# maxspahn/robot_mpcs

Measured on AMD Instinct MI355X. Metric: MPC solves/sec (batched) at N=30, pointRobot & panda; 1/2/4/8 MI355X, higher is better.
Workload: dtype f64; 1 GPU; BASELINE configs[1]: pointRobot N=30, batch=4096 random start/goal + 3 static obstacles; batch_per_gpu=4096, horizon=30, nvar=9, npar=38, nh=15, warm_start=current_state (cold multipliers, every step solves from scratch), parallelism=1 x independent shards, no data-path collective, streams_per_gpu=4, input_sets=6

## Files before the change

robot_mpcs_amd/csrc/rmpc_fused.hpp:

```cpp

constexpr int kFusedStages = 32;

struct FusedWs {
  double *p;
  double *z[2], *t[2], *lam[2], *nu[2];
  double *dz, *nunew, *gfa;
  double *grow[2], *Jq[2];
  double *wlam, *wnu, *wmu;
  double *R;
  double *KP;
  int *passes;
  int *lastp;
  int *order;
  int *ckey;
  long long *stamps;
  int rs, kps, nv, m, nx, npar, nhs, njqs;
};

#define GSYNC()                                              \
  do {                                                       \
    __builtin_amdgcn_fence(__ATOMIC_RELEASE, "wavefront");   \
    __builtin_amdgcn_s_waitcnt(0);                           \
    __builtin_amdgcn_wave_barrier();                         \
    __builtin_amdgcn_fence(__ATOMIC_ACQUIRE, "wavefront");   \
  } while (0)

#define RMPC_ONE_WAVE
#define RMPC_PHASE __noinline__ RMPC_ONE_WAVE
template <class C>
__device__ RMPC_PHASE bool fused_recursion_lds(const int N, const double dt, const double mu, const double cw, const int lane,
                                               ldouble *const work, ldouble *const slots, const StepOut<ldouble> so) {
  return riccati_recursion<C, kFusedStages, true, ldouble>(N, dt, mu, cw, lane, work, slots, nullptr, 0, so, slots);
}
template <class C>
__device__ RMPC_PHASE bool fused_recursion_mem(const int N, const double dt, const double mu, const double cw, const int lane,
                                               ldouble *const work, const gdouble *const grec, gdouble *const kpb,
                                               const int kps, const StepOut<gdouble> so) {
  return riccati_recursion<C, kFusedStages, false, gdouble, true>(N, dt, mu, cw, lane, work, grec, kpb, kps, so);
}

struct FusedPtrs {
  gdouble *pz[2], *pt[2], *pl[2], *pn[2], *pg[2], *pj[2], *pp, *pdz, *pnn, *pgf, *pwl, *pwn;
};
__device__ __forceinline__ FusedPtrs fused_ptrs(const FusedWs &F, size_t b) {
  asm volatile("" : "+v"(b));
  const size_t S = kFusedStages;
  FusedPtrs P;
  P.pz[0] = (gdouble *)F.z[0] + b * F.nv * S; P.pz[1] = (gdouble *)F.z[1] + b * F.nv * S;
  P.pt[0] = (gdouble *)F.t[0] + b * F.m * S; P.pt[1] = (gdouble *)F.t[1] + b * F.m * S;
  P.pl[0] = (gdouble *)F.lam[0] + b * F.m * S; P.pl[1] = (gdouble *)F.lam[1] + b * F.m * S;
  P.pn[0] = (gdouble *)F.nu[0] + b * F.nx * S; P.pn[1] = (gdouble *)F.nu[1] + b * F.nx * S;
  P.pg[0] = (gdouble *)F.grow[0] + b * F.nhs * S; P.pg[1] = (gdouble *)F.grow[1] + b * F.nhs * S;
  P.pj[0] = (gdouble *)F.Jq[0] + b * F.njqs * S; P.pj[1] = (gdouble *)F.Jq[1] + b * F.njqs * S;
  P.pp = (gdouble *)F.p + b * F.npar * S;
  P.pdz = (gdouble *)F.dz + b * F.nv * S;
  P.pnn = (gdouble *)F.nunew + b * F.nx * S;
  P.pgf = (gdouble *)F.gfa + b * F.nv * S;
  P.pwl = (gdouble *)F.wlam + b * F.m * S;
  P.pwn = (gdouble *)F.wnu + b * F.nx * S;
  return P;
}

typedef const __attribute__((address_space(4))) FusedWs cFusedWs;
__device__ __forceinline__ cFusedWs *uniform_block(const FusedWs *p) {
  const unsigned long long a = (unsigned long long)p;
  const unsigned lo = __builtin_amdgcn_readfirstlane((unsigned)a), hi = __builtin_amdgcn_readfirstlane((unsigned)(a >> 32));
  return (cFusedWs *)(((unsigned long long)hi << 32) | lo);
}
__device__ __forceinline__ void load_block(FusedWs &F, const FusedWs *p) {
  static_assert(sizeof(FusedWs) % 8 == 0, "FusedWs is copied in 8-byte words");
  const __attribute__((address_space(4))) unsigned long long *src = (const __attribute__((address_space(4))) unsigned long long *)uniform_block(p);
  unsigned long long *dst = (unsigned long long *)&F;
#pragma unroll
  for (int i = 0; i < (int)(sizeof(FusedWs) / 8); i++) dst[i] = src[i];
}
struct FusedCur {
  gdouble *zc, *zn, *tc, *tn, *lc, *ln, *nc, *nn, *gc, *gn, *jc, *jn, *pp, *pdz, *pnn, *pgf, *pwl, *pwn;
};
__device__ __forceinline__ FusedCur fused_cur(const FusedWs &F, const size_t b, const int cur) {
  const FusedPtrs P = fused_ptrs(F, b);
  const bool c1 = cur != 0;
  FusedCur Q;
  Q.zc = c1 ? P.pz[1] : P.pz[0]; Q.zn = c1 ? P.pz[0] : P.pz[1];
  Q.tc = c1 ? P.pt[1] : P.pt[0]; Q.tn = c1 ? P.pt[0] : P.pt[1];
  Q.lc = c1 ? P.pl[1] : P.pl[0]; Q.ln = c1 ? P.pl[0] : P.pl[1];
  Q.nc = c1 ? P.pn[1] : P.pn[0]; Q.nn = c1 ? P.pn[0] : P.pn[1];
  Q.gc = c1 ? P.pg[1] : P.pg[0]; Q.gn = c1 ? P.pg[0] : P.pg[1];
  Q.jc = c1 ? P.pj[1] : P.pj[0]; Q.jn = c1 ? P.pj[0] : P.pj[1];
  Q.pp = P.pp; Q.pdz = P.pdz; Q.pnn = P.pnn; Q.pgf = P.pgf; Q.pwl = P.pwl; Q.pwn = P.pwn;
  return Q;
}

struct ArmBlock {
  FusedWs F;
  DevModel M;
};
typedef const __attribute__((address_space(4))) ArmBlock cArmBlock;
struct FusedHalf {
  double gphi_sum;
  int b, valid, retired, first, ipass, nextslot;
};
template <class V>
__device__ __forceinline__ V call_view(const FusedWs *Fp) {
  if constexpr (std::is_same<V, GView>::value) {
    const unsigned long long a = (unsigned long long)Fp;
    const unsigned lo = (unsigned)__builtin_amdgcn_readfirstlane((unsigned)a), hi = (unsigned)__builtin_amdgcn_readfirstlane((unsigned)(a >> 32));
    const unsigned long long u = ((unsigned long long)hi << 32) | lo;
    typedef const __attribute__((address_space(4))) ArmBlock cArmBlock;
    cArmBlock *const blk = (cArmBlock *)u;
    return GView(&blk->M, (GView::cTables *)(u - sizeof(DevTables)));
  } else {
    return V{};
  }
}
struct StepRes { double ap, ad, gp; };
template <class C, class V, int FIRSTC, bool REC_LDS>
__device__ __noinline__ RMPC_ONE_WAVE Partials fused_sweep_call(const FusedWs *Fp, const int N, const double dt, const int use_curv,
                                                  const size_t b, const int cur, const int k, ldouble *const slots,
                                                  const bool nostep, const double alpha, const double adual, const double mu,
                                                  const int warm) {
  using RP = typename std::conditional<REC_LDS, ldouble, gdouble>::type;
  constexpr int GS = FusedSlots<C>::GS, DZ_OFF = FusedSlots<C>::DZ_OFF, NV = C::NV;
  FusedWs F;
  load_block(F, Fp);
  const size_t S = kFusedStages;
  const FusedCur Pw = fused_cur(F, b, cur);
  SweepIO<RP> io;
  io.zc = Pw.zc; io.tc = Pw.tc; io.lc = Pw.lc; io.nc = Pw.nc;
  io.zn = Pw.zn; io.tn = Pw.tn; io.ln = Pw.ln; io.nn = Pw.nn;
  io.pp = Pw.pp; io.gro = Pw.gc; io.jqo = Pw.jc; io.grn = Pw.gn; io.jqn = Pw.jn;
  io.gfa = Pw.pgf;
  io.SS = S; io.loff = (unsigned)k; io.kstride = 1u;
  if constexpr (REC_LDS) {
    io.rec = slots + k * GS;
    io.dzp = slots + DZ_OFF; io.nup = slots + DZ_OFF + NV;
    io.SSd = 1; io.loffd = (unsigned)(k * GS); io.kstrided = (unsigned)GS;
  } else {
    io.rec = (gdouble *)F.R + (b * (size_t)N + k) * C::RS;
    io.dzp = Pw.pdz; io.nup = Pw.pnn;
    io.SSd = S; io.loffd = (unsigned)k; io.kstrided = 1u;
  }
  io.wl = Pw.pwl; io.wn = Pw.pwn; io.warm = warm;
  const SweepK sk = {N, dt, use_curv};
  const V v = call_view<V>(Fp);
  Partials q = {0, 0, 0, 0, 0, 0, 0, 0, 1e300, 0};
  sweep_body<C, -1, RP, V, FIRSTC>(sk, v, io, k, FIRSTC != 0, nostep, alpha, adual, mu, q);
  return q;
}
template <class C, class V, bool REC_LDS>
__device__ __noinline__ RMPC_ONE_WAVE StepRes fused_step_call(const FusedWs *Fp, const size_t b, const int cur, const int k,
                                                ldouble *const slots, const double mu) {
  using RP = typename std::conditional<REC_LDS, ldouble, gdouble>::type;
  constexpr int GS = FusedSlots<C>::GS, DZ_OFF = FusedSlots<C>::DZ_OFF;
  FusedWs F;
  load_block(F, Fp);
  const size_t S = kFusedStages;
  const FusedCur Ps = fused_cur(F, b, cur);
  StepIO<RP> io;
  io.zc = Ps.zc; io.tc = Ps.tc; io.lc = Ps.lc; io.grow = Ps.gc; io.Jq = Ps.jc;
  io.gfa = Ps.pgf;
  io.SS = S; io.loff = (unsigned)k;
  if constexpr (REC_LDS) { io.dz = slots + DZ_OFF; io.SSd = 1; io.loffd = (unsigned)(k * GS); }
  else { io.dz = Ps.pdz; io.SSd = S; io.loffd = (unsigned)k; }
  const V v = call_view<V>(Fp);
  StepRes r = {1.0, 1.0, 0.0};
  step_body<C, RP, V>(v, io, k, mu, r.ap, r.ad, r.gp);
  return r;
}

struct SweepStepOut { double f, th, lgs, sumc, badf, rstat, req, rineq, rcomp, minc, amin_p, amin_d, gphi;
#ifdef RMPC_STAMPS
  long long tk[6];
#endif
};
struct SweepStepRes { Partials q; double amin_p, amin_d, gphi; };
template <class C, class V, int FIRSTC>
__device__ __noinline__ RMPC_ONE_WAVE void fused_sweep_step_call(__attribute__((address_space(3))) SweepStepOut *const out,
                                                                 const FusedWs *Fp, const int N, const double dt, const int use_curv,
                                                           const size_t b, const int cur, const int k, ldouble *const slots,
                                                           const bool live, const bool nostep, const bool fresh, const int ls,
                                                           const double amin_p_in, const double amin_d_in, const double gphi_in,
                                                           const double mu, const int warm) {
  constexpr int GS = FusedSlots<C>::GS, DZ_OFF = FusedSlots<C>::DZ_OFF, NV = C::NV;
  FusedWs F;
  load_block(F, Fp);
  const size_t S = kFusedStages;
  const FusedCur Pw = fused_cur(F, b, cur);
  const V v{};
  SweepIO<ldouble> io;
  io.zc = Pw.zc; io.tc = Pw.tc; io.lc = Pw.lc; io.nc = Pw.nc;
  io.zn = Pw.zn; io.tn = Pw.tn; io.ln = Pw.ln; io.nn = Pw.nn;
  io.pp = Pw.pp; io.gro = Pw.gc; io.jqo = Pw.jc; io.grn = Pw.gn; io.jqn = Pw.jn;
  io.gfa = Pw.pgf;
  io.SS = S; io.loff = (unsigned)k; io.kstride = 1u;
  io.rec = slots + k * GS;
  io.dzp = slots + DZ_OFF; io.nup = slots + DZ_OFF + NV;
  io.SSd = 1; io.loffd = (unsigned)(k * GS); io.kstrided = (unsigned)GS;
  io.wl = Pw.pwl; io.wn = Pw.pwn; io.warm = warm;
  const SweepK sk = {N, dt, use_curv};
  SweepStepRes r;
  const Partials qn = {0, 0, 0, 0, 0, 0, 0, 0, 1e300, 0};
  r.q = qn;
  SecStamps st;
  st.start();
  if constexpr (FIRSTC != 0) {
    r.amin_p = amin_p_in; r.amin_d = amin_d_in; r.gphi = gphi_in;
    if (live) sweep_body<C, -1, ldouble, V, FIRSTC>(sk, v, io, k, true, nostep, 0.0, 0.0, mu, r.q);
  } else {
    SweepTop<C, V> top;
    StepRow<C> sl;
    if (live) sweep_body<C, -1, ldouble, V, 0, 1>(sk, v, io, k, false, nostep, 0.0, 0.0, mu, r.q, nullptr, &top, &sl);
    double ap = (fresh && live) ? sl.ap : 1.0, ad = (fresh && live) ? sl.ad : 1.0, gp = (fresh && live) ? sl.gphi : 0.0;
    st(4);
    {
      double rs1[1] = {gp}, rm0[1] = {0.0}, rn2[2] = {ap, ad};
      wave_reduce_many<kFusedStages>(rs1, rm0, rn2);
      gp = rs1[0]; ap = rn2[0]; ad = rn2[1];
    }
    st(5);
    r.amin_p = fresh ? fmin(amin_p_in, ap) : amin_p_in;
    r.amin_d = fresh ? fmin(amin_d_in, ad) : amin_d_in;
    r.gphi = fresh ? gp : gphi_in;
    const double alpha = nostep ? 0.0 : ldexp(r.amin_p, -ls), adual = nostep ? 0.0 : r.amin_d;
    if (live) sweep_body<C, -1, ldouble, V, 0, 2>(sk, v, io, k, false, nostep, alpha, adual, mu, r.q, nullptr, &top);
  }
  {
    const Partials &q = r.q;
    double rs5[5] = {q.f, q.th, q.logs, q.sumc, q.bad}, rm4[4] = {q.rstat, q.req, q.rineq, q.rcomp}, rn1[1] = {q.minc};
    wave_reduce_many<kFusedStages>(rs5, rm4, rn1);
    out->f = rs5[0]; out->th = rs5[1]; out->lgs = rs5[2]; out->sumc = rs5[3]; out->badf = rs5[4];
    out->rstat = rm4[0]; out->req = rm4[1]; out->rineq = rm4[2]; out->rcomp = rm4[3]; out->minc = rn1[0];
    out->amin_p = r.amin_p; out->amin_d = r.amin_d; out->gphi = r.gphi;
    st.get(q, 0, 4);
    if (k == 0) st.put(*out, 0, 6);
  }
}

template <class C, bool REC_LDS, class V>
__global__ __launch_bounds__(64, 1) __attribute__((amdgpu_waves_per_eu(1, 1), disable_tail_calls)) void k_fused(const DevModel M, const DevTables *__restrict__ Tp, const FusedWs F, const int B,
                                              const double *__restrict__ xinit, const double *__restrict__ x0,
                                              const double *__restrict__ params, double *__restrict__ zout,
                                              int *__restrict__ exitflag, int *__restrict__ iters_out,
                                              double *__restrict__ kkt, double *__restrict__ obj, const int max_passes,
                                              const int warm_mode, const int use_order, const int save_duals) {
  constexpr int LPI = kFusedStages;
  constexpr int IPW = 2;
  constexpr int NX = C::NX, NV = C::NV;
  using VC = typename std::conditional<V::SPEC, V, GView>::type;
  auto blk = [&]() __attribute__((always_inline)) -> cArmBlock * {
    unsigned long long a = (unsigned long long)(Tp + 1);
    asm volatile("" : "+s"(a));
    return (cArmBlock *)a;
  };
  const int half = threadIdx.x / LPI;
  const int k = threadIdx.x & (LPI - 1);
  const int N = blk()->M.N;
  const bool stage = k < N;

  constexpr int LW = RicLds<C, LPI>::LDSW;
  constexpr int GS = FusedSlots<C>::GS;
  constexpr int DZ_OFF = FusedSlots<C>::DZ_OFF;
  constexpr int RECW = REC_LDS ? kFusedStages * GS : 0;
  __shared__ double lds[IPW * (LW + RECW)];
  ldouble *const work = (ldouble *)lds + half * (LW + RECW);
  ldouble *const slots = work + LW;

  const size_t S = kFusedStages;
  __shared__ Inst sinst[IPW];
  __shared__ FusedHalf shalf[IPW];
  __shared__ SweepStepOut sres[IPW];
  Inst s;
  const bool warm = warm_mode != 0;
  inst_init(s, blk()->M.mu0);
  s.status = 0;
  int bi = B - 1;
  bool valid = false;
  bool retired = false;
  bool first = true;
  int ipass = 0;
  int nextslot = blockIdx.x * IPW + half;
  double gphi_sum = 0.0;
  auto park = [&]() __attribute__((always_inline)) {
    if (k == 0) {
      sinst[half] = s;
      FusedHalf hw;
      hw.gphi_sum = gphi_sum; hw.b = bi; hw.ipass = ipass; hw.nextslot = nextslot;
      hw.valid = valid ? 1 : 0; hw.retired = retired ? 1 : 0; hw.first = first ? 1 : 0;
      shalf[half] = hw;
    }
  };
  auto unpark = [&]() __attribute__((always_inline)) {
    WSYNC();
    s = sinst[half];
    const FusedHalf hw = shalf[half];
    gphi_sum = hw.gphi_sum; bi = hw.b; ipass = hw.ipass; nextslot = hw.nextslot;
    valid = hw.valid != 0; retired = hw.retired != 0; first = hw.first != 0;
  };

  PassStamps ps;
  ps.start();
  for (;;) {
    ps.hand_begin();
    {
      const bool over = valid && (s.status == ST_ACTIVE) && ipass >= max_passes;
      const bool done = valid && (s.status != ST_ACTIVE || over);
      if (__ballot(done || (!valid && !retired)) != 0ull) {
        cArmBlock *const A = blk();
        const bool take = (done || !valid) && !retired;
        bool took = false;
        int qt = 0;
        if (take && nextslot < 0 && k == 0) qt = atomicAdd(A->F.passes + 1, 1);
        if (done) {
          const size_t b = (size_t)bi;
          const bool c1 = s.cur != 0;
          const bool okd = (s.status == ST_ACTIVE || s.status >= 0) && isfinite(s.mu) && s.mu > 0.0;
          if (stage) {
            const gdouble *zf = (const gdouble *)(c1 ? A->F.z[1] : A->F.z[0]) + b * A->F.nv * S;
            double *zr = zout + (b * N + k) * NV;
            double zv[NV];
#pragma unroll
            for (int j = 0; j < NV; j++) zv[j] = zf[j * S + k];
            if (save_duals) {
              const int m = A->F.m;
              const gdouble *lf = (const gdouble *)(c1 ? A->F.lam[1] : A->F.lam[0]) + b * m * S;
              const gdouble *nf = (const gdouble *)(c1 ? A->F.nu[1] : A->F.nu[0]) + b * A->F.nx * S;
              gdouble *wl = (gdouble *)A->F.wlam + b * m * S, *wn = (gdouble *)A->F.wnu + b * A->F.nx * S;
              double nv6[NX];
#pragma unroll
              for (int j = 0; j < NX; j++) nv6[j] = nf[j * S + k];
              constexpr int kDualSet = 36;
              for (int i0 = 0; i0 < m; i0 += kDualSet) {
                double lv[kDualSet];
#pragma unroll
                for (int u = 0; u < kDualSet; u++) lv[u] = lf[min(i0 + u, m - 1) * S + k];
                if (i0 == 0) {
#pragma unroll
                  for (int j = 0; j < NV; j++) zr[j] = zv[j];
#pragma unroll
                  for (int j = 0; j < NX; j++) wn[j * S + k] = okd ? nv6[j] : 0.0;
                }
#pragma unroll
                for (int u = 0; u < kDualSet; u++) wl[min(i0 + u, m - 1) * S + k] = okd ? lv[u] : 0.0;
              }
              if (m <= 0) {
#pragma unroll
                for (int j = 0; j < NV; j++) zr[j] = zv[j];
#pragma unroll
                for (int j = 0; j < NX; j++) wn[j * S + k] = okd ? nv6[j] : 0.0;
              }
            } else {
#pragma unroll
              for (int j = 0; j < NV; j++) zr[j] = zv[j];
            }
          }
          if (k == 0) {
            exitflag[b] = (s.status == ST_ACTIVE) ? 0 : s.status;
            iters_out[b] = s.iters;
            kkt[b] = fmax(fmax(s.res_stat, s.res_eq), fmax(s.res_ineq, s.res_comp));
            obj[b] = s.obj;
            if (save_duals) {
              A->F.wmu[b] = okd ? s.mu : A->M.mu0;
              A->F.lastp[b] = ipass;
            }
            atomicMax(A->F.passes, ipass);
          }
          valid = false;
          s.status = 0;
        }
        if (take) {
          int pos = nextslot;
          if (pos < 0) pos = (int)gridDim.x * IPW + __shfl(qt, half * LPI, 64);
          nextslot = -1;
          if (pos < B) {
            bi = use_order ? A->F.order[pos] : pos;
            const size_t b = (size_t)bi;
            valid = true;
            took = true;
            if (stage) {
              gdouble *const pz0 = (gdouble *)A->F.z[0] + b * A->F.nv * S;
              const double *zr = x0 + (b * N + k) * NV;
              double zv[NV];
#pragma unroll
              for (int j = 0; j < NV; j++) zv[j] = zr[j];
              if (k == 0) {
#pragma unroll
                for (int j = 0; j < NX; j++) zv[j] = xinit[b * NX + j];
              }
              if (params) {
                const int npar = A->M.npar;
                gdouble *const pp = (gdouble *)A->F.p + b * A->F.npar * S;
                const double *pr = params + (b * N + k) * npar;
                const int head = (int)(((unsigned long long)pr >> 3) & 1ull);
                const int np2 = (npar - head) >> 1;
                const bool tail = ((npar - head) & 1) != 0;
                const double h0 = head ? pr[0] : 0.0, t0 = tail ? pr[npar - 1] : 0.0;
                const double2 *pq = (const double2 *)(pr + head);
                constexpr int kParSet = 20;
                for (int j0 = 0; j0 < np2; j0 += kParSet) {
                  double2 pv[kParSet];
#pragma unroll
                  for (int u = 0; u < kParSet; u++) pv[u] = pq[min(j0 + u, np2 - 1)];
                  if (j0 == 0) {
#pragma unroll
                    for (int j = 0; j < NV; j++) pz0[j * S + k] = zv[j];
                  }
#pragma unroll
                  for (int u = 0; u < kParSet; u++) {
                    const int j = head + 2 * min(j0 + u, np2 - 1);
                    pp[j * S + k] = pv[u].x; pp[(j + 1) * S + k] = pv[u].y;
                  }
                }
                if (np2 <= 0) {
#pragma unroll
                  for (int j = 0; j < NV; j++) pz0[j * S + k] = zv[j];
                }
                if (head) pp[k] = h0;
                if (tail) pp[(npar - 1) * S + k] = t0;
              } else {
#pragma unroll
                for (int j = 0; j < NV; j++) pz0[j * S + k] = zv[j];
              }
              if constexpr (REC_LDS) {
#pragma unroll
                for (int j = 0; j < NV + NX; j++) slots[k * GS + DZ_OFF + j] = 0.0;
              }
            }
            {
              const double mu0 = A->M.mu0;
              inst_init(s, warm ? warm_mu(A->F.wmu[b], mu0) : mu0);
            }
            first = true;
            ipass = 0;
            gphi_sum = 0.0;
          } else {
            retired = true;
            bi = B - 1;
          }
        }
        GSYNC();
        ps.hand_events(done && k == 0, took && k == 0);
      }
    }
    const bool act = valid && (s.status == ST_ACTIVE);
    ps.hand_end();
    if (__ballot(act) == 0ull) break;
    if (act) ipass++;
    const bool v1 = act ? first : (__ballot(act && first) != 0ull);
    ps.pass_begin(act && k == 0, v1);
    ps.mark();
    Partials q = {0, 0, 0, 0, 0, 0, 0, 0, 1e300, 0};
    constexpr bool MERGE2 = V::SPEC && REC_LDS;
    park();
    bool fresh = false;
    if constexpr (MERGE2) {
      const bool nostep = first || (s.redo != 0);
      fresh = act && !nostep && (s.newstep != 0);
      const FusedWs *const Fp = (const FusedWs *)(Tp + 1);
      __attribute__((address_space(3))) SweepStepOut *const so = (__attribute__((address_space(3))) SweepStepOut *)&sres[half];
      cArmBlock *const A = blk();
      const double dt = A->M.dt;
      const int use_curv = A->M.use_curv;
      if (v1) fused_sweep_step_call<C, V, 1>(so, Fp, N, dt, use_curv, (size_t)bi, s.cur, k, slots, act && stage, nostep, fresh, s.ls, s.amin_p, s.amin_d, gphi_sum, s.mu, warm ? 1 : 0);
      else fused_sweep_step_call<C, V, 0>(so, Fp, N, dt, use_curv, (size_t)bi, s.cur, k, slots, act && stage, nostep, fresh, s.ls, s.amin_p, s.amin_d, gphi_sum, s.mu, warm ? 1 : 0);
    } else {
      if (act && stage) {
        const bool nostep = first || (s.redo != 0);
        double alpha = 0.0, adual = 0.0;
        if (!nostep) {
          alpha = ldexp(s.amin_p, -s.ls);
          adual = s.amin_d;
        }
        const FusedWs *const Fp = (const FusedWs *)(Tp + 1);
        cArmBlock *const A = blk();
        const double dt = A->M.dt;
        const int use_curv = A->M.use_curv;
        if (first) q = fused_sweep_call<C, VC, 1, REC_LDS>(Fp, N, dt, use_curv, (size_t)bi, s.cur, k, slots, nostep, alpha, adual, s.mu, warm ? 1 : 0);
        else q = fused_sweep_call<C, VC, 0, REC_LDS>(Fp, N, dt, use_curv, (size_t)bi, s.cur, k, slots, nostep, alpha, adual, s.mu, warm ? 1 : 0);
      }
    }
    ps.sweep_returned();
    unpark();
    Reduced r;
    if constexpr (MERGE2) {
      const SweepStepOut o = sres[half];
      if (fresh) { s.amin_p = o.amin_p; s.amin_d = o.amin_d; gphi_sum = o.gphi; }
      r.f = o.f; r.th = o.th; r.lgs = o.lgs; r.sumc = o.sumc; r.badf = o.badf;
      r.rstat = o.rstat; r.req = o.req; r.rineq = o.rineq; r.rcomp = o.rcomp; r.minc = o.minc;
      ps.sections(sres[half]);
    } else {
      ps.sections(q);
      double rs5[5] = {q.f, q.th, q.logs, q.sumc, q.bad}, rm4[4] = {q.rstat, q.req, q.rineq, q.rcomp}, rn1[1] = {q.minc};
      wave_reduce_many<LPI>(rs5, rm4, rn1);
      r.f = rs5[0]; r.th = rs5[1]; r.lgs = rs5[2]; r.sumc = rs5[3]; r.badf = rs5[4];
      r.rstat = rm4[0]; r.req = rm4[1]; r.rineq = rm4[2]; r.rcomp = rm4[3]; r.minc = rn1[0];
    }
    r.gphi = first ? 0.0 : gphi_sum;
    ps.sweep_reduced();
    GSYNC();
    ps.sweep_end();
    bool usec = false;
    bool recurse = false;
    if (act) recurse = inst_decide<C>(*(const DevModel *)&blk()->M, s, r, first, usec);
    if (act) first = false;
    ps(PH_DEC);
    park();
    const double mu_r = s.mu;
    const double cw_r = usec ? (C::CSCALE ? s.theta_c : 1.0) : 0.0;
    bool rec_ok = true;
    if (recurse) {
      bool ok;
      if constexpr (REC_LDS) {
        StepOut<ldouble> so;
        so.dz = slots + DZ_OFF; so.nunew = slots + DZ_OFF + NV; so.SS = 1; so.KS = GS;
        ok = fused_recursion_lds<C>(N, blk()->M.dt, mu_r, cw_r, k, work, slots, so);
      } else {
        cArmBlock *const A = blk();
        const size_t b = (size_t)bi;
        const int kps = A->F.kps;
        StepOut<gdouble> so;
        so.dz = (gdouble *)A->F.dz + b * A->F.nv * S; so.nunew = (gdouble *)A->F.nunew + b * A->F.nx * S; so.SS = S; so.KS = 1;
        ok = fused_recursion_mem<C>(N, A->M.dt, mu_r, cw_r, k, work, (gdouble *)A->F.R + b * (size_t)N * C::RS,
                                    (gdouble *)A->F.KP + b * (size_t)N * kps, kps, so);
      }
      rec_ok = ok;
    }
    unpark();
    if (recurse) inst_after_recursion(s, rec_ok, usec, C::BACKOFF, C::CSCALE);
    GSYNC();
    ps(PH_RIC);
    if constexpr (!MERGE2) {
      double ap = 1.0, ad = 1.0, gp = 0.0;
      const bool stepping = act && (s.status == ST_ACTIVE) && (s.newstep != 0);
      park();
      if (stepping && stage) {
        const FusedWs *const Fp = (const FusedWs *)(Tp + 1);
        const StepRes sr = fused_step_call<C, VC, REC_LDS>(Fp, (size_t)bi, s.cur, k, slots, s.mu);
        ap = sr.ap; ad = sr.ad; gp = sr.gp;
      }
      unpark();
      {
        double rs1[1] = {gp}, rm0[1] = {0.0}, rn2[2] = {ap, ad};
        wave_reduce_many<LPI>(rs1, rm0, rn2);
        gp = rs1[0]; ap = rn2[0]; ad = rn2[1];
      }
      if (stepping) {
        s.amin_p = fmin(s.amin_p, ap);
        s.amin_d = fmin(s.amin_d, ad);
        gphi_sum = gp;
      }
    }
    ps(PH_STEP);
  }
  ps.store(((cArmBlock *)(Tp + 1))->F.stamps, true);
}
```

robot_mpcs_amd/csrc/rmpc_stamps.hpp:

```cpp

enum StampPhase { PH_SWEEP = 0, PH_DEC = 1, PH_RIC = 2, PH_STEP = 3 };
#ifdef RMPC_STAMPS
static __device__ long long g_sst[8];
#endif
#if defined(RMPC_STAMPS) && !defined(RMPC_STAMPS_CALLS_ONLY)
struct SecStamps {
  long long acc[8], t0;
  __device__ __forceinline__ void start() {
    for (int i = 0; i < 8; i++) acc[i] = 0;
    t0 = __builtin_amdgcn_s_memtime();
  }
  __device__ __forceinline__ void operator()(const int i) {
    const long long t = __builtin_amdgcn_s_memtime();
    acc[i] += t - t0;
    t0 = t;
  }
  template <class O>
  __device__ __forceinline__ void put(O &o, const int i0, const int n) const {
    for (int i = i0; i < i0 + n; i++) o.tk[i] = acc[i];
  }
  template <class O>
  __device__ __forceinline__ void get(const O &o, const int i0, const int n) {
    for (int i = i0; i < i0 + n; i++) acc[i] = o.tk[i];
  }
  __device__ __forceinline__ void flush(const bool lane0, const int n) {
    if (lane0) {
      for (int i = 0; i < n; i++) atomicAdd((unsigned long long *)&g_sst[i], (unsigned long long)acc[i]);
      atomicAdd((unsigned long long *)&g_sst[7], 1ull);
    }
  }
};
#else
struct SecStamps {
  __device__ __forceinline__ void start() {}
  __device__ __forceinline__ void operator()(int) {}
  template <class O> __device__ __forceinline__ void put(O &, int, int) const {}
  template <class O> __device__ __forceinline__ void get(const O &, int, int) {}
  __device__ __forceinline__ void flush(bool, int) {}
};
#endif
#ifdef RMPC_STAMPS
struct PassStamps {
  long long ph[4], sec[8], hand, t_start, t_a, t_top, t_sub;
  int pass, ipass, nhand, both;
  __device__ __forceinline__ void start() {
    for (int i = 0; i < 4; i++) ph[i] = 0;
    for (int i = 0; i < 8; i++) sec[i] = 0;
    hand = 0;
    pass = ipass = nhand = both = 0;
    t_start = t_a = __builtin_amdgcn_s_memtime();
  }
  __device__ __forceinline__ void hand_begin() { t_top = __builtin_amdgcn_s_memtime(); }
  __device__ __forceinline__ void hand_events(const bool left, const bool took) {
    nhand += __popcll(__ballot(left)) + __popcll(__ballot(took));
  }
  __device__ __forceinline__ void hand_end() { hand += __builtin_amdgcn_s_memtime() - t_top; }
  __device__ __forceinline__ void pass_begin(const bool inst, const bool v1) {
    pass++;
    ipass += __popcll(__ballot(inst));
    both += (__ballot(v1) != 0ull && __ballot(!v1) != 0ull) ? 1 : 0;
  }
  __device__ __forceinline__ void mark() { t_a = __builtin_amdgcn_s_memtime(); }
  __device__ __forceinline__ void operator()(const int p) {
    const long long t = __builtin_amdgcn_s_memtime();
    ph[p] += t - t_a;
    t_a = t;
  }
  template <class O>
  __device__ __forceinline__ void sections(const O o) {
#ifndef RMPC_STAMPS_CALLS_ONLY
    for (int i = 0; i < 6; i++) sec[i] += __builtin_amdgcn_readfirstlane((int)o.tk[i]);
#endif
  }
  __device__ __forceinline__ void sweep_returned() { t_sub = __builtin_amdgcn_s_memtime(); }
  __device__ __forceinline__ void sweep_reduced() {
    const long long t = __builtin_amdgcn_s_memtime();
    sec[6] += t - t_sub;
    t_sub = t;
  }
  __device__ __forceinline__ void sweep_end() {
    (*this)(PH_SWEEP);
    sec[7] += t_a - t_sub;
  }
  __device__ __forceinline__ void store(long long *const stamps, const bool two) {
    if (threadIdx.x == 0) {
      long long *o = stamps + (size_t)blockIdx.x * 8;
      if (two) {
        long long *o2 = stamps + (size_t)(gridDim.x + blockIdx.x) * 8;
        for (int i = 0; i < 8; i++) o2[i] = sec[i];
      }
      for (int i = 0; i < 4; i++) o[i] = ph[i];
      o[4] = __builtin_amdgcn_s_memtime() - t_start;
      o[5] = (long long)pass | ((long long)both << 32);
      o[6] = two ? hand : t_start;
      o[7] = (long long)ipass | ((long long)nhand << 32);
    }
  }
};
#else
struct PassStamps {
  __device__ __forceinline__ void start() {}
  __device__ __forceinline__ void hand_begin() {}
  __device__ __forceinline__ void hand_events(bool, bool) {}
  __device__ __forceinline__ void hand_end() {}
  __device__ __forceinline__ void pass_begin(bool, bool) {}
  __device__ __forceinline__ void mark() {}
  __device__ __forceinline__ void operator()(int) {}
  template <class O> __device__ __forceinline__ void sections(O) {}
  __device__ __forceinline__ void sweep_returned() {}
  __device__ __forceinline__ void sweep_reduced() {}
  __device__ __forceinline__ void sweep_end() {}
  __device__ __forceinline__ void store(long long *, bool) {}
};
#endif
```

Baseline: 4.376 million solves/s.

## Refill finished instance slots mid-pass with an immediate second sweep round

Wraps the handoff and sweep in a two-round loop. When an instance finishes after the decision step, the wave grabs a new instance and runs its first sweep right away, instead of waiting for the next full pass, so lanes do not sit idle through the Riccati and step phases. Recurse and usec state is now carried through park/unpark, and the stepping condition uses valid instead of act. The extra round adds control flow, register pressure and a second sweep call per pass when instances retire, and changes per-lane phase alignment. Stamp counters are extended to count these early refills.

```diff
diff --git a/robot_mpcs_amd/csrc/rmpc_fused.hpp b/robot_mpcs_amd/csrc/rmpc_fused.hpp
--- a/robot_mpcs_amd/csrc/rmpc_fused.hpp
+++ b/robot_mpcs_amd/csrc/rmpc_fused.hpp
@@ -99,6 +99,7 @@
 struct FusedHalf {
   double gphi_sum;
   int b, valid, retired, first, ipass, nextslot;
+  int recurse, usec;
 };
 template <class V>
 __device__ __forceinline__ V call_view(const FusedWs *Fp) {
@@ -280,12 +281,15 @@
   int ipass = 0;
   int nextslot = blockIdx.x * IPW + half;
   double gphi_sum = 0.0;
+  bool recurse = false;
+  bool usec = false;
   auto park = [&]() __attribute__((always_inline)) {
     if (k == 0) {
       sinst[half] = s;
       FusedHalf hw;
       hw.gphi_sum = gphi_sum; hw.b = bi; hw.ipass = ipass; hw.nextslot = nextslot;
       hw.valid = valid ? 1 : 0; hw.retired = retired ? 1 : 0; hw.first = first ? 1 : 0;
+      hw.recurse = recurse ? 1 : 0; hw.usec = usec ? 1 : 0;
       shalf[half] = hw;
     }
   };
@@ -295,214 +299,225 @@
     const FusedHalf hw = shalf[half];
     gphi_sum = hw.gphi_sum; bi = hw.b; ipass = hw.ipass; nextslot = hw.nextslot;
     valid = hw.valid != 0; retired = hw.retired != 0; first = hw.first != 0;
+    recurse = hw.recurse != 0; usec = hw.usec != 0;
   };
 
+  constexpr bool MERGE2 = V::SPEC && REC_LDS;
   PassStamps ps;
   ps.start();
   for (;;) {
-    ps.hand_begin();
-    {
-      const bool over = valid && (s.status == ST_ACTIVE) && ipass >= max_passes;
-      const bool done = valid && (s.status != ST_ACTIVE || over);
-      if (__ballot(done || (!valid && !retired)) != 0ull) {
-        cArmBlock *const A = blk();
-        const bool take = (done || !valid) && !retired;
-        bool took = false;
-        int qt = 0;
-        if (take && nextslot < 0 && k == 0) qt = atomicAdd(A->F.passes + 1, 1);
-        if (done) {
-          const size_t b = (size_t)bi;
-          const bool c1 = s.cur != 0;
-          const bool okd = (s.status == ST_ACTIVE || s.status >= 0) && isfinite(s.mu) && s.mu > 0.0;
-          if (stage) {
-            const gdouble *zf = (const gdouble *)(c1 ? A->F.z[1] : A->F.z[0]) + b * A->F.nv * S;
-            double *zr = zout + (b * N + k) * NV;
-            double zv[NV];
-#pragma unroll
-            for (int j = 0; j < NV; j++) zv[j] = zf[j * S + k];
-            if (save_duals) {
-              const int m = A->F.m;
-              const gdouble *lf = (const gdouble *)(c1 ? A->F.lam[1] : A->F.lam[0]) + b * m * S;
-              const gdouble *nf = (const gdouble *)(c1 ? A->F.nu[1] : A->F.nu[0]) + b * A->F.nx * S;
-              gdouble *wl = (gdouble *)A->F.wlam + b * m * S, *wn = (gdouble *)A->F.wnu + b * A->F.nx * S;
-              double nv6[NX];
-#pragma unroll
-              for (int j = 0; j < NX; j++) nv6[j] = nf[j * S + k];
-              constexpr int kDualSet = 36;
-              for (int i0 = 0; i0 < m; i0 += kDualSet) {
-                double lv[kDualSet];
-#pragma unroll
-                for (int u = 0; u < kDualSet; u++) lv[u] = lf[min(i0 + u, m - 1) * S + k];
-                if (i0 == 0) {
+    bool idle = false;
+    recurse = false;
+    usec = false;
+#pragma nounroll
+    for (int round = 0;; round = 1) {
+      ps.hand_begin();
+      bool took = false;
+      {
+        const bool over = round == 0 && valid && (s.status == ST_ACTIVE) && ipass >= max_passes;
+        const bool done = valid && (s.status != ST_ACTIVE || over);
+        if (__ballot(done || (!valid && !retired)) != 0ull) {
+          cArmBlock *const A = blk();
+          const bool take = (done || !valid) && !retired;
+          int qt = 0;
+          if (take && nextslot < 0 && k == 0) qt = atomicAdd(A->F.passes + 1, 1);
+          if (done) {
+            const size_t b = (size_t)bi;
+            const bool c1 = s.cur != 0;
+            const bool okd = (s.status == ST_ACTIVE || s.status >= 0) && isfinite(s.mu) && s.mu > 0.0;
+            if (stage) {
+              const gdouble *zf = (const gdouble *)(c1 ? A->F.z[1] : A->F.z[0]) + b * A->F.nv * S;
+              double *zr = zout + (b * N + k) * NV;
+              double zv[NV];
+#pragma unroll
+              for (int j = 0; j < NV; j++) zv[j] = zf[j * S + k];
+              if (save_duals) {
+                const int m = A->F.m;
+                const gdouble *lf = (const gdouble *)(c1 ? A->F.lam[1] : A->F.lam[0]) + b * m * S;
+                const gdouble *nf = (const gdouble *)(c1 ? A->F.nu[1] : A->F.nu[0]) + b * A->F.nx * S;
+                gdouble *wl = (gdouble *)A->F.wlam + b * m * S, *wn = (gdouble *)A->F.wnu + b * A->F.nx * S;
+                double nv6[NX];
+#pragma unroll
+                for (int j = 0; j < NX; j++) nv6[j] = nf[j * S + k];
+                constexpr int kDualSet = 36;
+                for (int i0 = 0; i0 < m; i0 += kDualSet) {
+                  double lv[kDualSet];
+#pragma unroll
+                  for (int u = 0; u < kDualSet; u++) lv[u] = lf[min(i0 + u, m - 1) * S + k];
+                  if (i0 == 0) {
+#pragma unroll
+                    for (int j = 0; j < NV; j++) zr[j] = zv[j];
+#pragma unroll
+                    for (int j = 0; j < NX; j++) wn[j * S + k] = okd ? nv6[j] : 0.0;
+                  }
+#pragma unroll
+                  for (int u = 0; u < kDualSet; u++) wl[min(i0 + u, m - 1) * S + k] = okd ? lv[u] : 0.0;
+                }
+                if (m <= 0) {
 #pragma unroll
                   for (int j = 0; j < NV; j++) zr[j] = zv[j];
 #pragma unroll
                   for (int j = 0; j < NX; j++) wn[j * S + k] = okd ? nv6[j] : 0.0;
                 }
-#pragma unroll
-                for (int u = 0; u < kDualSet; u++) wl[min(i0 + u, m - 1) * S + k] = okd ? lv[u] : 0.0;
+              } else {
+#pragma unroll
+                for (int j = 0; j < NV; j++) zr[j] = zv[j];
               }
-              if (m <= 0) {
-#pragma unroll
-                for (int j = 0; j < NV; j++) zr[j] = zv[j];
-#pragma unroll
-                for (int j = 0; j < NX; j++) wn[j * S + k] = okd ? nv6[j] : 0.0;
+            }
+            if (k == 0) {
+              exitflag[b] = (s.status == ST_ACTIVE) ? 0 : s.status;
+              iters_out[b] = s.iters;
+              kkt[b] = fmax(fmax(s.res_stat, s.res_eq), fmax(s.res_ineq, s.res_comp));
+              obj[b] = s.obj;
+              if (save_duals) {
+                A->F.wmu[b] = okd ? s.mu : A->M.mu0;
+                A->F.lastp[b] = ipass;
               }
+              atomicMax(A->F.passes, ipass);
+            }
+            valid = false;
+            s.status = 0;
+          }
+          if (take) {
+            int pos = nextslot;
+            if (pos < 0) pos = (int)gridDim.x * IPW + __shfl(qt, half * LPI, 64);
+            nextslot = -1;
+            if (pos < B) {
+              bi = use_order ? A->F.order[pos] : pos;
+              const size_t b = (size_t)bi;
+              valid = true;
+              took = true;
+              if (stage) {
+                gdouble *const pz0 = (gdouble *)A->F.z[0] + b * A->F.nv * S;
+                const double *zr = x0 + (b * N + k) * NV;
+                double zv[NV];
+#pragma unroll
+                for (int j = 0; j < NV; j++) zv[j] = zr[j];
+                if (k == 0) {
+#pragma unroll
+                  for (int j = 0; j < NX; j++) zv[j] = xinit[b * NX + j];
+                }
+                if (params) {
+                  const int npar = A->M.npar;
+                  gdouble *const pp = (gdouble *)A->F.p + b * A->F.npar * S;
+                  const double *pr = params + (b * N + k) * npar;
+                  const int head = (int)(((unsigned long long)pr >> 3) & 1ull);
+                  const int np2 = (npar - head) >> 1;
+                  const bool tail = ((npar - head) & 1) != 0;
+                  const double h0 = head ? pr[0] : 0.0, t0 = tail ? pr[npar - 1] : 0.0;
+                  const double2 *pq = (const double2 *)(pr + head);
+                  constexpr int kParSet = 20;
+                  for (int j0 = 0; j0 < np2; j0 += kParSet) {
+                    double2 pv[kParSet];
+#pragma unroll
+                    for (int u = 0; u < kParSet; u++) pv[u] = pq[min(j0 + u, np2 - 1)];
+                    if (j0 == 0) {
+#pragma unroll
+                      for (int j = 0; j < NV; j++) pz0[j * S + k] = zv[j];
+                    }
+#pragma unroll
+                    for (int u = 0; u < kParSet; u++) {
+                      const int j = head + 2 * min(j0 + u, np2 - 1);
+                      pp[j * S + k] = pv[u].x; pp[(j + 1) * S + k] = pv[u].y;
+                    }
+                  }
+                  if (np2 <= 0) {
+#pragma unroll
+                    for (int j = 0; j < NV; j++) pz0[j * S + k] = zv[j];
+                  }
+                  if (head) pp[k] = h0;
+                  if (tail) pp[(npar - 1) * S + k] = t0;
+                } else {
+#pragma unroll
+                  for (int j = 0; j < NV; j++) pz0[j * S + k] = zv[j];
+                }
+                if constexpr (REC_LDS) {
+#pragma unroll
+                  for (int j = 0; j < NV + NX; j++) slots[k * GS + DZ_OFF + j] = 0.0;
+                }
+              }
+              {
+                const double mu0 = A->M.mu0;
+                inst_init(s, warm ? warm_mu(A->F.wmu[b], mu0) : mu0);
+              }
+              first = true;
+              ipass = 0;
+              gphi_sum = 0.0;
             } else {
-#pragma unroll
-              for (int j = 0; j < NV; j++) zr[j] = zv[j];
+              retired = true;
+              bi = B - 1;
             }
           }
-          if (k == 0) {
-            exitflag[b] = (s.status == ST_ACTIVE) ? 0 : s.status;
-            iters_out[b] = s.iters;
-            kkt[b] = fmax(fmax(s.res_stat, s.res_eq), fmax(s.res_ineq, s.res_comp));
-            obj[b] = s.obj;
-            if (save_duals) {
-              A->F.wmu[b] = okd ? s.mu : A->M.mu0;
-              A->F.lastp[b] = ipass;
-            }
-            atomicMax(A->F.passes, ipass);
-          }
-          valid = false;
-          s.status = 0;
+          GSYNC();
+          ps.hand_events(done && k == 0, took && k == 0, round);
         }
-        if (take) {
-          int pos = nextslot;
-          if (pos < 0) pos = (int)gridDim.x * IPW + __shfl(qt, half * LPI, 64);
-          nextslot = -1;
-          if (pos < B) {
-            bi = use_order ? A->F.order[pos] : pos;
-            const size_t b = (size_t)bi;
-            valid = true;
-            took = true;
-            if (stage) {
-              gdouble *const pz0 = (gdouble *)A->F.z[0] + b * A->F.nv * S;
-              const double *zr = x0 + (b * N + k) * NV;
-              double zv[NV];
-#pragma unroll
-              for (int j = 0; j < NV; j++) zv[j] = zr[j];
-              if (k == 0) {
-#pragma unroll
-                for (int j = 0; j < NX; j++) zv[j] = xinit[b * NX + j];
-              }
-              if (params) {
-                const int npar = A->M.npar;
-                gdouble *const pp = (gdouble *)A->F.p + b * A->F.npar * S;
-                const double *pr = params + (b * N + k) * npar;
-                const int head = (int)(((unsigned long long)pr >> 3) & 1ull);
-                const int np2 = (npar - head) >> 1;
-                const bool tail = ((npar - head) & 1) != 0;
-                const double h0 = head ? pr[0] : 0.0, t0 = tail ? pr[npar - 1] : 0.0;
-                const double2 *pq = (const double2 *)(pr + head);
-                constexpr int kParSet = 20;
-                for (int j0 = 0; j0 < np2; j0 += kParSet) {
-                  double2 pv[kParSet];
-#pragma unroll
-                  for (int u = 0; u < kParSet; u++) pv[u] = pq[min(j0 + u, np2 - 1)];
-                  if (j0 == 0) {
-#pragma unroll
-                    for (int j = 0; j < NV; j++) pz0[j * S + k] = zv[j];
-                  }
-#pragma unroll
-                  for (int u = 0; u < kParSet; u++) {
-                    const int j = head + 2 * min(j0 + u, np2 - 1);
-                    pp[j * S + k] = pv[u].x; pp[(j + 1) * S + k] = pv[u].y;
-                  }
-                }
-                if (np2 <= 0) {
-#pragma unroll
-                  for (int j = 0; j < NV; j++) pz0[j * S + k] = zv[j];
-                }
-                if (head) pp[k] = h0;
-                if (tail) pp[(npar - 1) * S + k] = t0;
-              } else {
-#pragma unroll
-                for (int j = 0; j < NV; j++) pz0[j * S + k] = zv[j];
-              }
-              if constexpr (REC_LDS) {
-#pragma unroll
-                for (int j = 0; j < NV + NX; j++) slots[k * GS + DZ_OFF + j] = 0.0;
-              }
-            }
-            {
-              const double mu0 = A->M.mu0;
-              inst_init(s, warm ? warm_mu(A->F.wmu[b], mu0) : mu0);
-            }
-            first = true;
-            ipass = 0;
-            gphi_sum = 0.0;
-          } else {
-            retired = true;
-            bi = B - 1;
-          }
-        }
-        GSYNC();
-        ps.hand_events(done && k == 0, took && k == 0);
-      }
-    }
-    const bool act = valid && (s.status == ST_ACTIVE);
-    ps.hand_end();
-    if (__ballot(act) == 0ull) break;
-    if (act) ipass++;
-    const bool v1 = act ? first : (__ballot(act && first) != 0ull);
-    ps.pass_begin(act && k == 0, v1);
-    ps.mark();
-    Partials q = {0, 0, 0, 0, 0, 0, 0, 0, 1e300, 0};
-    constexpr bool MERGE2 = V::SPEC && REC_LDS;
-    park();
-    bool fresh = false;
-    if constexpr (MERGE2) {
-      const bool nostep = first || (s.redo != 0);
-      fresh = act && !nostep && (s.newstep != 0);
-      const FusedWs *const Fp = (const FusedWs *)(Tp + 1);
-      __attribute__((address_space(3))) SweepStepOut *const so = (__attribute__((address_space(3))) SweepStepOut *)&sres[half];
-      cArmBlock *const A = blk();
-      const double dt = A->M.dt;
-      const int use_curv = A->M.use_curv;
-      if (v1) fused_sweep_step_call<C, V, 1>(so, Fp, N, dt, use_curv, (size_t)bi, s.cur, k, slots, act && stage, nostep, fresh, s.ls, s.amin_p, s.amin_d, gphi_sum, s.mu, warm ? 1 : 0);
-      else fused_sweep_step_call<C, V, 0>(so, Fp, N, dt, use_curv, (size_t)bi, s.cur, k, slots, act && stage, nostep, fresh, s.ls, s.amin_p, s.amin_d, gphi_sum, s.mu, warm ? 1 : 0);
-    } else {
-      if (act && stage) {
+      }
+      const bool act = valid && (s.status == ST_ACTIVE) && (round == 0 || took);
+      ps.hand_end();
+      if (__ballot(act) == 0ull) {
+        idle = round == 0;
+        break;
+      }
+      if (act) ipass++;
+      const bool v1 = act ? first : (__ballot(act && first) != 0ull);
+      ps.pass_begin(act && k == 0, v1, round);
+      ps.mark();
+      Partials q = {0, 0, 0, 0, 0, 0, 0, 0, 1e300, 0};
+      park();
+      bool fresh = false;
+      if constexpr (MERGE2) {
         const bool nostep = first || (s.redo != 0);
-        double alpha = 0.0, adual = 0.0;
-        if (!nostep) {
-          alpha = ldexp(s.amin_p, -s.ls);
-          adual = s.amin_d;
-        }
+        fresh = act && !nostep && (s.newstep != 0);
         const FusedWs *const Fp = (const FusedWs *)(Tp + 1);
+        __attribute__((address_space(3))) SweepStepOut *const so = (__attribute__((address_space(3))) SweepStepOut *)&sres[half];
         cArmBlock *const A = blk();
         const double dt = A->M.dt;
         const int use_curv = A->M.use_curv;
-        if (first) q = fused_sweep_call<C, VC, 1, REC_LDS>(Fp, N, dt, use_curv, (size_t)bi, s.cur, k, slots, nostep, alpha, adual, s.mu, warm ? 1 : 0);
-        else q = fused_sweep_call<C, VC, 0, REC_LDS>(Fp, N, dt, use_curv, (size_t)bi, s.cur, k, slots, nostep, alpha, adual, s.mu, warm ? 1 : 0);
-      }
+        if (v1) fused_sweep_step_call<C, V, 1>(so, Fp, N, dt, use_curv, (size_t)bi, s.cur, k, slots, act && stage, nostep, fresh, s.ls, s.amin_p, s.amin_d, gphi_sum, s.mu, warm ? 1 : 0);
+        else fused_sweep_step_call<C, V, 0>(so, Fp, N, dt, use_curv, (size_t)bi, s.cur, k, slots, act && stage, nostep, fresh, s.ls, s.amin_p, s.amin_d, gphi_sum, s.mu, warm ? 1 : 0);
+      } else {
+        if (act && stage) {
+          const bool nostep = first || (s.redo != 0);
+          double alpha = 0.0, adual = 0.0;
+          if (!nostep) {
+            alpha = ldexp(s.amin_p, -s.ls);
+            adual = s.amin_d;
+          }
+          const FusedWs *const Fp = (const FusedWs *)(Tp + 1);
+          cArmBlock *const A = blk();
+          const double dt = A->M.dt;
+          const int use_curv = A->M.use_curv;
+          if (first) q = fused_sweep_call<C, VC, 1, REC_LDS>(Fp, N, dt, use_curv, (size_t)bi, s.cur, k, slots, nostep, alpha, adual, s.mu, warm ? 1 : 0);
+          else q = fused_sweep_call<C, VC, 0, REC_LDS>(Fp, N, dt, use_curv, (size_t)bi, s.cur, k, slots, nostep, alpha, adual, s.mu, warm ? 1 : 0);
+        }
+      }
+      ps.sweep_returned();
+      unpark();
+      Reduced r;
+      if constexpr (MERGE2) {
+        const SweepStepOut o = sres[half];
+        if (fresh) { s.amin_p = o.amin_p; s.amin_d = o.amin_d; gphi_sum = o.gphi; }
+        r.f = o.f; r.th = o.th; r.lgs = o.lgs; r.sumc = o.sumc; r.badf = o.badf;
+        r.rstat = o.rstat; r.req = o.req; r.rineq = o.rineq; r.rcomp = o.rcomp; r.minc = o.minc;
+        ps.sections(sres[half]);
+      } else {
+        ps.sections(q);
+        double rs5[5] = {q.f, q.th, q.logs, q.sumc, q.bad}, rm4[4] = {q.rstat, q.req, q.rineq, q.rcomp}, rn1[1] = {q.minc};
+        wave_reduce_many<LPI>(rs5, rm4, rn1);
+        r.f = rs5[0]; r.th = rs5[1]; r.lgs = rs5[2]; r.sumc = rs5[3]; r.badf = rs5[4];
+        r.rstat = rm4[0]; r.req = rm4[1]; r.rineq = rm4[2]; r.rcomp = rm4[3]; r.minc = rn1[0];
+      }
+      r.gphi = first ? 0.0 : gphi_sum;
+      ps.sweep_reduced();
+      GSYNC();
+      ps.sweep_end();
+      if (act) recurse = inst_decide<C>(*(const DevModel *)&blk()->M, s, r, first, usec);
+      if (act) first = false;
+      ps(PH_DEC);
+      if (round != 0 || __ballot(valid && s.status != ST_ACTIVE) == 0ull) break;
     }
-    ps.sweep_returned();
-    unpark();
-    Reduced r;
-    if constexpr (MERGE2) {
-      const SweepStepOut o = sres[half];
-      if (fresh) { s.amin_p = o.amin_p; s.amin_d = o.amin_d; gphi_sum = o.gphi; }
-      r.f = o.f; r.th = o.th; r.lgs = o.lgs; r.sumc = o.sumc; r.badf = o.badf;
-      r.rstat = o.rstat; r.req = o.req; r.rineq = o.rineq; r.rcomp = o.rcomp; r.minc = o.minc;
-      ps.sections(sres[half]);
-    } else {
-      ps.sections(q);
-      double rs5[5] = {q.f, q.th, q.logs, q.sumc, q.bad}, rm4[4] = {q.rstat, q.req, q.rineq, q.rcomp}, rn1[1] = {q.minc};
-      wave_reduce_many<LPI>(rs5, rm4, rn1);
-      r.f = rs5[0]; r.th = rs5[1]; r.lgs = rs5[2]; r.sumc = rs5[3]; r.badf = rs5[4];
-      r.rstat = rm4[0]; r.req = rm4[1]; r.rineq = rm4[2]; r.rcomp = rm4[3]; r.minc = rn1[0];
-    }
-    r.gphi = first ? 0.0 : gphi_sum;
-    ps.sweep_reduced();
-    GSYNC();
-    ps.sweep_end();
-    bool usec = false;
-    bool recurse = false;
-    if (act) recurse = inst_decide<C>(*(const DevModel *)&blk()->M, s, r, first, usec);
-    if (act) first = false;
-    ps(PH_DEC);
+    if (idle) break;
+    ps.mark();
     park();
     const double mu_r = s.mu;
     const double cw_r = usec ? (C::CSCALE ? s.theta_c : 1.0) : 0.0;
@@ -530,7 +545,7 @@
     ps(PH_RIC);
     if constexpr (!MERGE2) {
       double ap = 1.0, ad = 1.0, gp = 0.0;
-      const bool stepping = act && (s.status == ST_ACTIVE) && (s.newstep != 0);
+      const bool stepping = valid && (s.status == ST_ACTIVE) && (s.newstep != 0);
       park();
       if (stepping && stage) {
         const FusedWs *const Fp = (const FusedWs *)(Tp + 1);
diff --git a/robot_mpcs_amd/csrc/rmpc_stamps.hpp b/robot_mpcs_amd/csrc/rmpc_stamps.hpp
--- a/robot_mpcs_amd/csrc/rmpc_stamps.hpp
+++ b/robot_mpcs_amd/csrc/rmpc_stamps.hpp
@@ -42,22 +42,24 @@
 #ifdef RMPC_STAMPS
 struct PassStamps {
   long long ph[4], sec[8], hand, t_start, t_a, t_top, t_sub;
-  int pass, ipass, nhand, both;
+  int pass, ipass, nhand, both, nearly;
   __device__ __forceinline__ void start() {
     for (int i = 0; i < 4; i++) ph[i] = 0;
     for (int i = 0; i < 8; i++) sec[i] = 0;
     hand = 0;
-    pass = ipass = nhand = both = 0;
+    pass = ipass = nhand = both = nearly = 0;
     t_start = t_a = __builtin_amdgcn_s_memtime();
   }
   __device__ __forceinline__ void hand_begin() { t_top = __builtin_amdgcn_s_memtime(); }
-  __device__ __forceinline__ void hand_events(const bool left, const bool took) {
+  __device__ __forceinline__ void hand_events(const bool left, const bool took, const int round = 0) {
     nhand += __popcll(__ballot(left)) + __popcll(__ballot(took));
+    if (round != 0) nearly += __popcll(__ballot(left));
   }
   __device__ __forceinline__ void hand_end() { hand += __builtin_amdgcn_s_memtime() - t_top; }
-  __device__ __forceinline__ void pass_begin(const bool inst, const bool v1) {
+  __device__ __forceinline__ void pass_begin(const bool inst, const bool v1, const int round = 0) {
+    ipass += __popcll(__ballot(inst));
+    if (round != 0) return;
     pass++;
-    ipass += __popcll(__ballot(inst));
     both += (__ballot(v1) != 0ull && __ballot(!v1) != 0ull) ? 1 : 0;
   }
   __device__ __forceinline__ void mark() { t_a = __builtin_amdgcn_s_memtime(); }
@@ -91,7 +93,7 @@
       }
       for (int i = 0; i < 4; i++) o[i] = ph[i];
       o[4] = __builtin_amdgcn_s_memtime() - t_start;
-      o[5] = (long long)pass | ((long long)both << 32);
+      o[5] = (long long)pass | ((long long)(both & 0xffff) << 32) | ((long long)(nearly & 0xffff) << 48);
       o[6] = two ? hand : t_start;
       o[7] = (long long)ipass | ((long long)nhand << 32);
     }
@@ -101,9 +103,9 @@
 struct PassStamps {
   __device__ __forceinline__ void start() {}
   __device__ __forceinline__ void hand_begin() {}
-  __device__ __forceinline__ void hand_events(bool, bool) {}
+  __device__ __forceinline__ void hand_events(bool, bool, int = 0) {}
   __device__ __forceinline__ void hand_end() {}
-  __device__ __forceinline__ void pass_begin(bool, bool) {}
+  __device__ __forceinline__ void pass_begin(bool, bool, int = 0) {}
   __device__ __forceinline__ void mark() {}
   __device__ __forceinline__ void operator()(int) {}
   template <class O> __device__ __forceinline__ void sections(O) {}
```

Measured after the change: 4.451 million solves/s (median of 6 runs). 1.7% higher.
